# USDA-ARS-GBRU/itsxpress

Measured on AMD Instinct MI355X. Metric: reads/sec trimmed (ITS2, stand-in taxon Tracheophyta for Fungi), higher is better.
Workload: dtype u8+f32

## Files before the change

itsxpress_amd/csrc/engine.hip:

```cpp
#include <algorithm>
#include <chrono>
#include <cmath>
#include <cstdio>
#include <cstring>
#include <functional>
#include <map>
#include <memory>
#include <numeric>
#include <atomic>
#include <condition_variable>
#include <mutex>
#include <thread>
#include "detmath.h"
#include "engine.h"
#include "k_api.h"
#include "cluster_multi.h"
#include "fastq_io.h"
#include "writers.h"

namespace itsx {
void launch_region_offsets(int64_t npairs, const PairRec *pairs, const int32_t *pref, const int64_t *seg_pair_start,
                           const int64_t *seg_region_start, int64_t *pair_region0, hipStream_t st);
void launch_finalize(itsx_domain *dom, int64_t n, const int64_t *domz, double domE, const int32_t *usample, int P, hipStream_t st);
void launch_positions(const itsx_domain *dom, int64_t n, const int8_t *side, unsigned long long *bl, unsigned long long *br,
// ... 2233 lines not shown
      const int lanes_norm = waves_target <= 0 ? MR_LANES : (int)std::max<int64_t>(2, std::min<int64_t>(MR_LANES, (NU + waves_target - 1) / waves_target));
      std::vector<WaveDesc> mw;
      std::vector<int64_t> wfirst;
      for (int64_t x = 0; x < NU;) {
        const int lanes = x >= NU - n_long ? std::min(lanes_long, lanes_norm) : (int)std::min<int64_t>(lanes_norm, NU - n_long - x);
        WaveDesc d{};
        d.prof = -1; d.first = x; d.count = (int32_t)std::min<int64_t>(lanes, (int64_t)NU - x);
        d.rows = hlen[(size_t)ord[(size_t)(d.first + d.count - 1)]] + 1;
        wfirst.push_back(x);
        mw.push_back(d);
        x += d.count;
      }
      const int NMW = (int)mw.size();
      wfirst.push_back(NU);
      HIPCHK(upload(ctx->w_mrwaves, mw, st));
      const int64_t mrow_bytes = (int64_t)MRV * 16;
      const int64_t mbudget = std::max<int64_t>(1, (int64_t)(std::min(slab_gb, 16.0) * (1 << 30)) / mrow_bytes);
      const int64_t wave_cap = std::max<int64_t>(1, ((int64_t)6 << 30) / ((int64_t)MR_SCRATCH * MR_LANES));
      int w0 = 0;
      int64_t mr_wave_cap = wave_cap;
      while (w0 < NMW) {
        int w1 = w0;
        const int64_t row0 = hrow[(size_t)wfirst[(size_t)w0]];
        auto rows_to = [&](int w) { return hrow[(size_t)wfirst[(size_t)std::min(w, NMW)]] - row0; };
        while (w1 < NMW && w1 - w0 < std::min(wave_cap, mr_wave_cap) && (w1 == w0 || rows_to(w1 + 1) <= mbudget)) w1++;
        const int64_t r = rows_to(w1);
        if (((size_t)r * MRV * 4 > ctx->w_mrslab.cap && ctx->w_mrslab.alloc((size_t)r * MRV * 4) != hipSuccess) ||
            ctx->w_mrscratch.alloc((size_t)(wfirst[(size_t)w1] - wfirst[(size_t)w0]) * MR_SCRATCH) != hipSuccess) {
          (void)hipGetLastError();
          if (w1 - w0 <= 1) SET_ERR(ctx, ITSX_E_NOMEM, "no device memory left for the matrices of one wave of multidomain regions");
          mr_wave_cap = std::max<int64_t>(1, (int64_t)(w1 - w0) / 2);
          S.n_slab_shrinks++;
          continue;
        }
        MrArgs ma{};
        ma.rd = ctx->rd; ma.sorted_uniq = d_sorted; ma.seed_read = ctx->d_seed_read.p; ma.prof = ctx->d_prof.p; ma.pairs = pl.pairs;
        ma.mr = ctx->w_mr.p; ma.ulist = ulist.p; ma.u0 = wfirst[(size_t)w0]; ma.waves = ctx->w_mrwaves.p; ma.slab = (float4 *)ctx->w_mrslab.p;
        ma.rowoff = ctx->w_mrrowoff.p; ma.rowoff0 = row0;
        ma.n2off = ctx->w_n2off.p; ma.n2sc = ctx->w_n2sc.p; ma.out = ctx->w_mrout.p; ma.scratch = ctx->w_mrscratch.p;
        static const bool mrdbg = sw_get("ITSX_MR_DEBUG") != nullptr;
        if (mrdbg) { HIPCHK(ctx->w_counters.alloc(8)); HIPCHK(hipMemsetAsync(ctx->w_counters.p, 0, 64, st)); ma.dbg = (unsigned long long *)ctx->w_counters.p; }
        const int64_t one_max = sw_get("ITSX_MR_ONE_MAX") ? atoll(sw_get("ITSX_MR_ONE_MAX")) : 2048;
        const int64_t nreg = wfirst[(size_t)w1] - wfirst[(size_t)w0];
        const bool one = nreg <= one_max;
        if (one) ma.lds_bytes = (int32_t)std::min<int64_t>(40 << 10, (int64_t)mw[(size_t)w1 - 1].rows * MRV * 16);
        launch_mr_ensemble(ma, w1 - w0, w0, st, one ? wfirst[(size_t)w0] : 0, one ? nreg : 0);
        if (mrdbg) {
          unsigned long long d[5];
          HIPCHK(hipMemcpyAsync(d, ctx->w_counters.p, 40, hipMemcpyDeviceToHost, st)); HIPCHK(hipStreamSynchronize(st));
          fprintf(stderr, "[itsx] ensemble batch: %d waves, %lld matrix rows; per wave (100 MHz ticks): walk %.0f, close %.0f (samples %.0f), cluster %.0f\n", w1 - w0, (long long)r,
                  (double)d[0] / std::max<double>(1.0, (double)d[3]), (double)d[1] / std::max<double>(1.0, (double)d[3]), (double)d[4] / std::max<double>(1.0, (double)d[3]),
                  (double)d[2] / std::max<double>(1.0, (double)d[3]));
        }
        w0 = w1;
      }
      {
        HIPCHK(ctx->w_mrsel.alloc((size_t)NU + 1)); HIPCHK(ctx->w_pool_n.alloc(2));
        HIPCHK(hipMemsetAsync(ctx->w_pool_n.p + 1, 0, sizeof(unsigned long long), st));
        launch_mr_overflowed(ctx->w_mrout.p, NU, ctx->w_mrsel.p, ctx->w_pool_n.p + 1, st);
        unsigned long long nov = 0;
        HIPCHK(hipMemcpyAsync(&nov, ctx->w_pool_n.p + 1, sizeof(nov), hipMemcpyDeviceToHost, st));
        HIPCHK(hipStreamSynchronize(st));
        if (nov > 0) {
          std::vector<int32_t> sel((size_t)nov);
          HIPCHK(hipMemcpyAsync(sel.data(), ctx->w_mrsel.p, (size_t)nov * 4, hipMemcpyDeviceToHost, st));
// ... 18 lines not shown
              const int64_t bytes = al(8ll * g.capT) + 6 * al(4ll * g.capT) + al(4ll * hs) + al(4ll * g.capD) + al(16ll * g.capD) + 3 * al(4 * capSig) +
                                    al(g.capT) + al(2ll * g.capD) + al(capSig) + al(2 * MR_EPC) + 64;
              g.envoff = envoff[x1];
              if (x1 > x0 && arena + bytes > ((int64_t)8 << 30)) break;
              g.off = arena; arena += bytes;
              big.push_back(g); srow.push_back(rows); rows += Lr + 1;
              x1++;
            }
            for (size_t x = x0; x < x1; x += MR_LANES_LONG) {
              WaveDesc d{}; d.prof = -1; d.first = (int64_t)(x - x0); d.count = (int32_t)std::min<size_t>(MR_LANES_LONG, x1 - x);
              d.rows = hlen[(size_t)ord[(size_t)sel[x + d.count - 1]]] + 1;
              bw.push_back(d);
            }
            std::vector<int32_t> selb(sel.begin() + x0, sel.begin() + x1);
            HIPCHK(upload(ctx->w_mrsel, selb, st)); HIPCHK(upload(ctx->w_mrselrow, srow, st)); HIPCHK(upload(ctx->w_mrbig, big, st)); HIPCHK(upload(ctx->w_mrbigwaves, bw, st));
            if ((size_t)rows * MRV * 4 > ctx->w_mrslab.cap) HIPCHK(ctx->w_mrslab.alloc((size_t)rows * MRV * 4));
            HIPCHK(ctx->w_mrarena.alloc((size_t)arena));
            MrArgs mb{};
            mb.rd = ctx->rd; mb.sorted_uniq = d_sorted; mb.seed_read = ctx->d_seed_read.p; mb.prof = ctx->d_prof.p; mb.pairs = pl.pairs;
            mb.mr = ctx->w_mr.p; mb.ulist = ulist.p; mb.u0 = 0; mb.waves = ctx->w_mrbigwaves.p; mb.slab = (float4 *)ctx->w_mrslab.p;
            mb.rowoff = ctx->w_mrrowoff.p; mb.rowoff0 = 0; mb.n2off = ctx->w_n2off.p; mb.n2sc = ctx->w_n2sc.p; mb.out = ctx->w_mrout.p;
            mb.scratch = nullptr; mb.sel = ctx->w_mrsel.p; mb.sel_rowoff = ctx->w_mrselrow.p; mb.big = ctx->w_mrbig.p; mb.arena = ctx->w_mrarena.p; mb.envpool = ctx->w_mrenv.p;
            launch_mr_ensemble_big(mb, (int)bw.size(), st);
            x0 = x1;
          }
        }
      }
      S.ms_ensemble += tm_e.stop();
      HIPCHK(hipGetLastError());
      S.n_mr_clustered += NMR; S.n_mr_distinct += NU;
    }
  }
  DBuf<int32_t> &d_rcnt = ctx->w_rcnt, &d_rpref = ctx->w_rpref, &d_scan_tmp = ctx->w_scan2;
  HIPCHK(d_rcnt.alloc((size_t)NP + 1)); HIPCHK(d_rpref.alloc((size_t)NP + 1)); HIPCHK(d_scan_tmp.alloc((size_t)scan_tmp_elems(NP + 1)));
  HIPCHK(hipMemsetAsync(d_rcnt.p, 0, ((size_t)NP + 1) * 4, st));
// ... 2015 lines not shown
```

itsxpress_amd/csrc/k_api.h:

```cpp
#pragma once
#include "engine.h"

#include "detmath.h"
namespace itsx {

struct ReadsDev {
  const uint32_t *words;
  const int64_t  *woff;
  const int32_t  *len;
  const int64_t  *excoff;
  const uint32_t *exc;
  int64_t         n;
};

void launch_hash_reads(const ReadsDev &rd, uint64_t seed, int strand_both, uint64_t *hf, uint64_t *hr, hipStream_t st, const int32_t *sample = nullptr);
void launch_table_insert(int64_t n, const int32_t *len, int minlen, const uint64_t *hf, const uint64_t *hr,
                         unsigned long long *keys, int32_t *vals, uint64_t mask, uint32_t *slot_of, hipStream_t st);
void launch_table_resolve(const ReadsDev &rd, const uint64_t *hf, const int32_t *vals, const uint32_t *slot_of,
                          int32_t *rep_of, int8_t *strand, int32_t *is_seed, unsigned int *n_collisions, hipStream_t st,
                          const int32_t *sample = nullptr);
void launch_uniques(int64_t n, const int32_t *rep_of, const int32_t *seed_rank, int32_t *uniq_of, int32_t *seed_read,
                    int32_t *abundance, hipStream_t st);
void launch_len_hist(int32_t U, const int32_t *seed_read, const int32_t *len, int32_t *hist, int32_t lcap, hipStream_t st, int32_t nb = 0 );
void launch_len_scatter(int32_t U, const int32_t *seed_read, const int32_t *len, int32_t *cursor, int32_t lcap,
// ... 307 lines not shown

struct EnvArgs {
  ReadsDev rd;
  const int32_t *sorted_uniq, *seed_read;
  const DevProfile *prof;
  const LenTables *lt;
  const PairRec *pairs;
  const RegionRec *regions;
  RegionOut *rout;
  const WaveDesc *waves;
  float *slab;
};
void launch_envelopes(const EnvArgs &a, int nwaves, int wave0, int generic_q, hipStream_t st);

constexpr int MRV = 52;
constexpr int MRENV = 4;
#ifndef ITSX_MR_LANES
#define ITSX_MR_LANES 64
#endif
constexpr int MR_LANES = ITSX_MR_LANES;
constexpr int MR_LANES_LONG = 4;
constexpr double MR_LONG_FRAC = 0.02;
constexpr int MR_MAXD = 8;
constexpr int MR_TCAP = 512;
constexpr int MR_SCAP = 200 * MR_MAXD;
constexpr int MR_NSIG = 32;
static_assert(MR_NSIG * 50 >= 200 * MR_MAXD, "MR_NSIG must hold every cluster that can reach 25 % of 200 paths");
constexpr int MR_HASH = 1024;
constexpr int MR_EPC = 256;
constexpr int MR_SCRATCH = 19456;
struct MrRec { int32_t pair, ireg, jreg, slot; };
struct MrOut { int32_t status, nenv; int32_t ei[MRENV], ej[MRENV]; int64_t big; };
struct MrBig { int64_t off, envoff; int32_t capD, capT; uint32_t hmask; int32_t pad; };
struct MrArgs {
  ReadsDev rd;
  const int32_t *sorted_uniq, *seed_read;
  const DevProfile *prof;
  const PairRec *pairs;
  const MrRec *mr;
  const int32_t *ulist;
  int64_t u0;
  const WaveDesc *waves;
  int32_t lds_bytes = 0;
  float4 *slab;
  const int64_t *rowoff;
  int64_t rowoff0;
  const int64_t *n2off;
  float *n2sc;
  MrOut *out;
  uint8_t *scratch;
  const int32_t *sel; const int64_t *sel_rowoff; const MrBig *big; uint8_t *arena;
  int32_t *envpool;
  unsigned long long *dbg;
};
void launch_mr_count(const PairOut *pout, const RegionRec *raw, RegionPoolView pv, int64_t npairs, int32_t *cnt, hipStream_t st);
void launch_mr_fill(const PairOut *pout, const RegionRec *raw, RegionPoolView pv, int64_t npairs, const int32_t *off, MrRec *mr, hipStream_t st);
void launch_mr_ulist(int64_t nmr, const MrRec *mr, const int32_t *rep, const int32_t *is_uniq, const int32_t *urank, int32_t *ulist, int32_t *ulen,
                     int32_t *mr_u, hipStream_t st);
void launch_mr_reorder(int64_t nu, int64_t nmr, const int32_t *newpos, const int32_t *ulist_in, int32_t *ulist_out, int32_t *mr_u, hipStream_t st);
// ... 72 lines not shown
```

itsxpress_amd/csrc/k_ensemble.hip:

```cpp
#include "engine.h"
#include "k_api.h"
#include "detmath.h"
#include "k_vec.h"
#include <type_traits>

namespace itsx {

enum { tBM = 0, tMM, tIM, tDM, tMD, tMI, tII, tDD };
enum { ST_M = 1, ST_D, ST_I, ST_S, ST_N, ST_B, ST_E, ST_C, ST_T, ST_J };

DEV f4 *mrslab(const MrArgs &a, int64_t r0, int row, int v, int lane) { (void)lane; return (f4 *)a.slab + ((r0 + row) * MRV + v); }
constexpr int MR_SP = QMAX * 4 + 1, MR_CJ = QMAX * 4 + 2;
static_assert(MR_CJ < MRV, "matrix row too short");
DEV float comp4(const f4 &t, int r) { return r == 0 ? t.x : r == 1 ? t.y : r == 2 ? t.z : t.w; }
DEV f4 tof4(const V4 &v) { return (f4){v.a.x, v.a.y, v.b.x, v.b.y}; }

struct MrLane {
  bool active; int64_t mi, slot; MrRec m; int L, Lr, off, Q; const DevProfile *pp; Seq sq; float pmove, ploop; int64_t r0;
};
DEV MrLane mr_lane(const MrArgs &a, const WaveDesc &wd, int lane)
{
  MrLane e;
  e.active = lane < wd.count;
  const int64_t slot = wd.first + (e.active ? lane : 0);
// ... 102 lines not shown

DEV uint32_t rnd_mix3(uint32_t a, uint32_t b, uint32_t c)
{
  a -= b; a -= c; a ^= (c >> 13);
  b -= c; b -= a; b ^= (a << 8);
  c -= a; c -= b; c ^= (b >> 13);
  a -= b; a -= c; a ^= (c >> 12);
  b -= c; b -= a; b ^= (a << 16);
  c -= a; c -= b; c ^= (b >> 5);
  a -= b; a -= c; a ^= (c >> 3);
  b -= c; b -= a; b ^= (a << 10);
  c -= a; c -= b; c ^= (b >> 15);
  return c;
}
DEV double rng_next(uint32_t &x) { x *= 69069u; x += 1u; return (double)x / 4294967296.0; }
DEV int choose_n(uint32_t &rng, int n, float p0, float p1, float p2, float p3)
{
  float sum = 0.f; sum += p0; sum += p1; sum += p2; sum += p3;
  if (sum != 0.0f) { p0 /= sum; p1 /= sum; p2 /= sum; p3 /= sum; }
  else { p0 = p1 = (float)(1. / (double)(float)n); p2 = p3 = n == 4 ? p0 : 0.0f; }
  const double roll = rng_next(rng);
  double s = 0.0;
  s += p0; if (roll < s) return 0;
  s += p1; if (roll < s) return 1;
  s += p2; if (roll < s) return 2;
  s += p3; if (roll < s) return 3;
  int i;
  do { i = (int)(rng_next(rng) * n); } while ((i == 0 ? p0 : i == 1 ? p1 : i == 2 ? p2 : p3) == 0.f);
  return i;
}

DEV int choose2(uint32_t &rng, float p0, float p1)
{
  float sum = 0.f; sum += p0; sum += p1;
  if (sum != 0.0f) { p0 /= sum; p1 /= sum; }
  else { p0 = p1 = (float)(1. / (double)(float)2); }
  const double roll = rng_next(rng);
  double s = 0.0;
  s += p0; if (roll < s) return 0;
  s += p1; if (roll < s) return 1;
  int i;
  do { i = (int)(rng_next(rng) * 2); } while ((i == 0 ? p0 : p1) == 0.f);
  return i;
}

struct Tup { int i, j, k, m; };
DEV Tup unpack_tup(unsigned long long v) { Tup t; t.i = (int)(v & 0xffff); t.j = (int)((v >> 16) & 0xffff); t.k = (int)((v >> 32) & 0xff); t.m = (int)((v >> 40) & 0xff); return t; }
DEV unsigned long long pack_tup(int i, int j, int k, int m) { return (unsigned long long)i | ((unsigned long long)j << 16) | ((unsigned long long)k << 32) | ((unsigned long long)m << 40); }
DEV bool link_tup(const Tup &h1, const Tup &h2)
{
  int nov = min(h1.j, h2.j) - max(h1.i, h2.i) + 1;
  int n = min(h1.j - h1.i + 1, h2.j - h2.i + 1);
  if ((float)nov / (float)n < 0.8f) return false;
  nov = min(h1.m, h2.m) - max(h1.k, h2.k);
  n = min(h1.m - h1.k + 1, h2.m - h2.k + 1);
  if ((float)nov / (float)n < 0.8f) return false;
  int d1 = h1.i - h1.k, d2 = h2.i - h2.k;
  if (abs(d1 - d2) <= 4) return true;
// ... 21 lines not shown
  constexpr idx_t NONE = (idx_t)~(idx_t)0;
  constexpr int NL = ONE ? 1 : MR_LANES;
  __shared__ uint16_t cntI_s[QMAX * 4][NL];
  __shared__ uint32_t dom_ij[MR_MAXD][NL];
  __shared__ uint16_t dom_km[MR_MAXD][NL];
  __shared__ f4 dn2_one[ONE ? MR_MAXD : 1];
  WaveDesc wd;
  if constexpr (ONE) { wd.prof = -1; wd.first = wave0 + (int64_t)(gridDim.x - 1 - blockIdx.x); wd.count = 1; wd.rows = 0; }
  else wd = a.waves[wave0 + (gridDim.x - 1 - blockIdx.x)];
  const bool coop = !ONE && !BIG && wd.count <= 8;
  int P2 = 1; while (P2 < wd.count) P2 <<= 1;
  const int G = coop ? 64 / P2 : 1, hlp = coop ? (int)threadIdx.x / P2 : 0;
  const int lane = ONE ? 0 : (coop ? (int)threadIdx.x % P2 : (int)threadIdx.x);
  const MrLane e = mr_lane(a, wd, lane);
  const f4 *mat = (const f4 *)a.slab + e.r0 * MRV;
  bool in_lds = false;
  if constexpr (ONE) {
    const int64_t nvec = (int64_t)(e.Lr + 1) * MRV;
    if (nvec * 16 <= (int64_t)a.lds_bytes) {
      for (int64_t z = threadIdx.x; z < nvec; z += 64) mr_mat[z] = mat[z];
      in_lds = true;
    }
    __syncthreads();
  } else {
    if (!e.active) return;
  }
  const bool walker = ONE ? threadIdx.x == 0 : hlp == 0;
  const int tid = (int)threadIdx.x;
#define MATV(idx) ((ONE && in_lds) ? mr_mat[(idx)] : mat[(idx)])
  const int Q = e.Q, Lr = e.Lr, Lw = ONE ? e.Lr : wd.rows - 1;
  const float *tfn = e.pp->tfn;
  const float pmove = e.pmove, ploop = e.ploop;
  float *n2 = a.n2sc + a.n2off[e.mi];
  MrBig bg; bg.off = 0; bg.envoff = 0; bg.capD = MR_MAXD; bg.capT = MR_TCAP; bg.hmask = MR_HASH - 1; bg.pad = 0;
  if constexpr (BIG) bg = a.big[e.slot];
  const int capD = BIG ? bg.capD : MR_MAXD, capT = BIG ? bg.capT : MR_TCAP, capS = BIG ? bg.capT : MR_SCAP;
  const int capSig = BIG ? 4 * bg.capD : MR_NSIG, capEnv = BIG ? 4 * bg.capD : MRENV;
  const uint32_t hmask = BIG ? bg.hmask : (uint32_t)(MR_HASH - 1);
  unsigned long long *Skey; idx_t *Stcount, *Scomp, *Sstack, *Sninc, *Stid, *Shslot; sidx_t *Slast; uint8_t *Stidx, *Sdominated;
  uint16_t *Sepc; int32_t *Ssig_i, *Ssig_j, *Senv = nullptr; float *Ssig_p; f4 *Sdn2; uint32_t *Gdom_ij = nullptr; uint16_t *Gdom_km = nullptr;
  if constexpr (BIG) {
    uint8_t *blk = a.arena + bg.off;
    size_t o = 0;
    auto take = [&](size_t bytes) { uint8_t *q = blk + o; o += (bytes + 15) & ~(size_t)15; return q; };
// ... 2 lines not shown
    Sninc = (idx_t *)take(4 * (size_t)capT); Slast = (sidx_t *)take(4 * (size_t)capT); Stid = (idx_t *)take(4 * (size_t)capT);
    Shslot = (idx_t *)take(4 * ((size_t)hmask + 1));
    Gdom_ij = (uint32_t *)take(4 * (size_t)capD); Sdn2 = (f4 *)take(16 * (size_t)capD);
    Ssig_i = (int32_t *)take(4 * (size_t)capSig); Ssig_j = (int32_t *)take(4 * (size_t)capSig); Ssig_p = (float *)take(4 * (size_t)capSig);
    Senv = a.envpool + bg.envoff;
    Stidx = (uint8_t *)take((size_t)capT); Gdom_km = (uint16_t *)take(2 * (size_t)capD); Sdominated = (uint8_t *)take((size_t)capSig);
    Sepc = (uint16_t *)take(2 * MR_EPC);
  } else {
    MrScratch &S = *(MrScratch *)(a.scratch + (int64_t)(e.mi - a.u0) * MR_SCRATCH);
    Skey = S.key; Stcount = (idx_t *)S.tcount; Scomp = (idx_t *)S.comp; Sstack = (idx_t *)S.stack; Sninc = (idx_t *)S.ninc; Slast = (sidx_t *)S.last;
    Stid = (idx_t *)S.tid; Stidx = S.tidx; Shslot = (idx_t *)S.hslot; Sepc = S.epc; Ssig_i = S.sig_i; Ssig_j = S.sig_j; Ssig_p = S.sig_p;
    Sdominated = S.dominated; Sdn2 = S.dn2;
  }
#define DOM_IJ(d) (*(BIG ? &Gdom_ij[(d)] : &dom_ij[(d) < MR_MAXD ? (d) : 0][lane]))
#define DOM_KM(d) (*(BIG ? &Gdom_km[(d)] : &dom_km[(d) < MR_MAXD ? (d) : 0][lane]))
  if constexpr (ONE) {
    for (int pos = tid; pos < Lr; pos += 64) n2[pos] = 0.0f;
    for (uint32_t z = (uint32_t)tid; z <= hmask; z += 64) Shslot[z] = 0;
    __threadfence_block();
    __syncthreads();
  } else if (coop) {
    for (int pos = hlp; pos < Lr; pos += G) n2[pos] = 0.0f;
    for (uint32_t z = (uint32_t)hlp; z <= hmask; z += (uint32_t)G) Shslot[z] = 0;
    __threadfence_block();
    __syncthreads();
  } else {
    for (int pos = 0; pos < Lr; pos++) n2[pos] = 0.0f;
    for (uint32_t z = 0; z <= hmask; z++) Shslot[z] = 0;
  }
  uint32_t rng = rnd_mix3(42u, 87654321u, 12345678u);
  if (rng == 0) rng = 42;
  int ntup = 0, nsamp = 0, status = walker ? 0 : 9;
  const unsigned short dgm[16] = {1, 2, 4, 8, 0, 5, 10, 3, 12, 6, 9, 11, 14, 7, 13, 15};
  int ex0p = -1, ex0c = 0, ex1p = -1, ex1c = 0;
  if (e.sq.nexc >= 1 && e.sq.nexc <= 2) { const uint32_t v = e.sq.exc[0]; ex0p = (int)(v >> 4); ex0c = (int)(v & 15u); }
  if (e.sq.nexc == 2) { const uint32_t v = e.sq.exc[1]; ex1p = (int)(v >> 4); ex1c = (int)(v & 15u); }

  unsigned long long tk_walk = 0, tk_close = 0, tk_dedupe = 0;
  for (int t = 0; t < 200; t++) {
    if (__ballot(status == 0) == 0ull) break;
    const unsigned long long tk0 = wall_clock64();
    int i = Lr, k = 0, s0 = status == 0 ? ST_C : ST_S, nd = 0;
    int cj_row = -1; f4 cj_cur = (f4){0.f, 0.f, 0.f, 0.f};
    int dfrom = 0, dto = 0, dk = 0, dm = 0;
    unsigned long long maskM = 0ull;
    while (__ballot(s0 != ST_S) != 0ull) {
      while (__ballot(s0 == ST_C || s0 == ST_J) != 0ull) {
        if (!(s0 == ST_C || s0 == ST_J)) continue;
        if (i < 1) { status = 5; s0 = ST_S; continue; }
        if (cj_row != i) { cj_cur = MATV((int64_t)i * MRV + MR_CJ); cj_row = i; }
        const f4 c0 = MATV((int64_t)(i - 1) * MRV + MR_CJ);
        const float w0 = (s0 == ST_C ? c0.z : c0.y) * ploop, w1 = cj_cur.x * 0.5f * cj_cur.w;
        if (choose2(rng, w0, w1) == 0) { i--; cj_cur = c0; cj_row = i; } else s0 = ST_E;
      }
      if (__ballot(s0 == ST_E) != 0ull) {
        if (s0 == ST_E) {
          double sum = 0.0;
          const double roll = rng_next(rng);
          const double norm = 1.0 / (double)cj_cur.x;
          const float xEv = (float)norm;
          int s1 = -1;
          while (s1 < 0) {
            for (int q0 = 0; q0 < Q && s1 < 0; q0 += 3) {
              f2 md[3][4];
#pragma unroll
              for (int z = 0; z < 3; z++) {
                const int qq = q0 + z < Q ? q0 + z : Q - 1;
#pragma unroll
                for (int rr = 0; rr < 4; rr++) { const f4 q4 = MATV((int64_t)i * MRV + (rr * Q + qq + 1)); md[z][rr] = (f2){q4.x, q4.y}; }
              }
#pragma unroll
              for (int z = 0; z < 3; z++) {
                if (q0 + z >= Q || s1 >= 0) continue;
                const int qq = q0 + z;
#pragma unroll
                for (int rr = 0; rr < 4; rr++) { if (s1 < 0) { sum += (double)(md[z][rr].x * xEv); if (roll < sum) { k = rr * Q + qq + 1; s1 = ST_M; } } }
// ... 4 lines not shown
            if (s1 < 0 && sum < 0.99) { status = 1; s1 = ST_S; }
          }
          if (status == 0 && nd >= capD) { status = 2; s1 = ST_S; }
          if (status == 0) {
            nd++;
            dfrom = dto = dk = dm = 0;
            maskM = 0ull;
            for (int z = 0; z < Q * 4; z++) cntI_s[z][lane] = 0;
            if (s1 == ST_M) { dto = i; dm = k; dfrom = i; dk = k; maskM |= 1ull << k; }
          }
          s0 = s1;
        }
      }
      while (__ballot(s0 == ST_M || s0 == ST_D || s0 == ST_I) != 0ull) {
        if (!(s0 == ST_M || s0 == ST_D || s0 == ST_I)) continue;
        const int rowA = (s0 == ST_D) ? i : i - 1;
        const int kA = (s0 == ST_I) ? k : k - 1;
        const f4 nv = MATV((int64_t)rowA * MRV + kA);
        const f4 tv = *(const f4 *)(tfn + (s0 == ST_D ? kA : k) * 8 + (s0 == ST_M ? 0 : 4));
        float w0, w1, w2 = 0.0f, w3 = 0.0f;
        if (s0 == ST_M) { w0 = nv.w * tv.x; w1 = nv.x * tv.y; w2 = nv.z * tv.z; w3 = nv.y * tv.w; }
        else if (s0 == ST_D) { w0 = nv.x * tv.x; w1 = nv.y * tv.w; }
        else { w0 = nv.x * tv.y; w1 = nv.z * tv.z; }
        const int c = choose_n(rng, s0 == ST_M ? 4 : 2, w0, w1, w2, w3);
        int s1;
        if (s0 == ST_M) { s1 = c == 0 ? ST_B : c == 1 ? ST_M : c == 2 ? ST_I : ST_D; k--; i--; }
        else if (s0 == ST_D) { s1 = c == 0 ? ST_M : ST_D; k--; }
        else { s1 = c == 0 ? ST_M : ST_I; i--; }
        if (s1 == ST_M) {
          if (dto == 0) { dto = i; dm = k; }
          dfrom = i; dk = k;
          maskM |= 1ull << k;
        } else if (s1 == ST_I) {
          cntI_s[k - 1][lane] += 1;
        }
        s0 = s1;
      }
      if (__ballot(s0 == ST_B) != 0ull) {
        if (s0 == ST_B) {
          const f4 sp1 = MATV((int64_t)i * MRV + MR_SP);
          s0 = choose2(rng, sp1.y * pmove, sp1.z * pmove) == 0 ? ST_S : ST_J;
          int Ld = __popcll(maskM);
          for (int z = 0; z < Q * 4; z++) Ld += (int)cntI_s[z][lane];
          const float norm = (float)(1.0 / (double)(float)Ld);
          const float xfactor = (0.0f * norm + 0.0f * norm) + 0.0f * norm;
          V4 sv[4];
#pragma unroll
          for (int x = 0; x < 4; x++) sv[x] = vzero();
          for (int qq = 0; qq < Q; qq++) {
            V4 mv, iv;
            mv.a = (f2){(float)((maskM >> (0 * Q + qq + 1)) & 1ull), (float)((maskM >> (1 * Q + qq + 1)) & 1ull)};
            mv.b = (f2){(float)((maskM >> (2 * Q + qq + 1)) & 1ull), (float)((maskM >> (3 * Q + qq + 1)) & 1ull)};
            iv.a = (f2){(float)cntI_s[0 * Q + qq][lane], (float)cntI_s[1 * Q + qq][lane]}; iv.b = (f2){(float)cntI_s[2 * Q + qq][lane], (float)cntI_s[3 * Q + qq][lane]};
            mv = vmul(mv, vset(norm)); iv = vmul(iv, vset(norm));
#pragma unroll
            for (int x = 0; x < 4; x++) {
// ... 267 lines not shown
      }
    for (int d = 0; d < nsig; d++) {
      if (Sdominated[d]) continue;
      if (out.nenv >= capEnv) { status = 7; break; }
      if (out.nenv < MRENV) { out.ei[out.nenv] = Ssig_i[d]; out.ej[out.nenv] = Ssig_j[d]; }
      if constexpr (BIG) { Senv[2 * out.nenv] = Ssig_i[d]; Senv[2 * out.nenv + 1] = Ssig_j[d]; }
      out.nenv++;
    }
  }
  if (status != 0) {
    out.nenv = 0;
    for (int pos = 0; pos < Lr; pos++) n2[pos] = 0.0f;
  }
  out.status = status;
  a.out[e.mi] = out;
  if (a.dbg && lane == 0) { atomicAdd(&a.dbg[0], tk_walk); atomicAdd(&a.dbg[1], tk_close); atomicAdd(&a.dbg[2], wall_clock64() - tk2); atomicAdd(&a.dbg[3], 1ull); atomicAdd(&a.dbg[4], tk_dedupe); }
}
#undef DOM_IJ
#undef DOM_KM

__global__ void __launch_bounds__(256) k_mr_count(const PairOut *__restrict__ pout, const RegionRec *__restrict__ raw, RegionPoolView pv, int64_t npairs,
                                                  int32_t *__restrict__ cnt)
{
  const int64_t pi = (int64_t)blockIdx.x * blockDim.x + threadIdx.x;
  if (pi > npairs) return;
  int c = 0;
  if (pi < npairs && pout[pi].pass_fwd)
    for (int k = 0; k < pout[pi].ndom; k++) c += raw_region(raw, pv, pi, k).multi != 0;
  cnt[pi] = c;
}
__global__ void __launch_bounds__(256) k_mr_fill(const PairOut *__restrict__ pout, const RegionRec *__restrict__ raw, RegionPoolView pv, int64_t npairs,
                                                 const int32_t *__restrict__ off, MrRec *__restrict__ mr)
{
  const int64_t pi = (int64_t)blockIdx.x * blockDim.x + threadIdx.x;
// ... 105 lines not shown
                     int32_t *mr_u, hipStream_t st)
{
  if (nmr <= 0) return;
  hipLaunchKernelGGL(k_mr_ulist, dim3((unsigned)((nmr + 255) / 256)), dim3(256), 0, st, nmr, mr, rep, is_uniq, urank, ulist, ulen, mr_u);
}
void launch_mr_reorder(int64_t nu, int64_t nmr, const int32_t *newpos, const int32_t *ulist_in, int32_t *ulist_out, int32_t *mr_u, hipStream_t st)
{
  const int64_t n = nu > nmr ? nu : nmr;
  if (n <= 0) return;
  hipLaunchKernelGGL(k_mr_reorder, dim3((unsigned)((n + 255) / 256)), dim3(256), 0, st, nu, nmr, newpos, ulist_in, ulist_out, mr_u);
}
void launch_mr_ensemble(const MrArgs &a, int nwaves, int wave0, hipStream_t st, int64_t one_first, int64_t one_count)
{
  if (nwaves <= 0) return;
  hipLaunchKernelGGL(k_mr_fwd, dim3(nwaves), dim3(64), 0, st, a, wave0);
  if (one_count > 0) hipLaunchKernelGGL((k_mr_trace<false, true>), dim3((unsigned)one_count), dim3(64), (size_t)a.lds_bytes, st, a, (int)one_first);
  else hipLaunchKernelGGL(k_mr_trace<false>, dim3(nwaves), dim3(64), 0, st, a, wave0);
}
void launch_mr_ensemble_big(const MrArgs &a, int nwaves, hipStream_t st)
{
  if (nwaves <= 0) return;
  hipLaunchKernelGGL(k_mr_fwd, dim3(nwaves), dim3(64), 0, st, a, 0);
  hipLaunchKernelGGL(k_mr_trace<true>, dim3(nwaves), dim3(64), 0, st, a, 0);
}
}
```

itsxpress_amd/csrc/switches.cpp:

```cpp
#include "switches.h"
#include <cstdlib>
#include <cstring>

namespace itsx {

static const Switch g_sw[] = {
  {"ITSX_NO_ENSEMBLE", SW_HOOK, "multidomain regions keep their region as one envelope instead of hmmsearch's stochastic-traceback clustering (changes envelopes)"},
  {"ITSX_LAZY_ZUB_SCALE", SW_HOOK, "multiplies the lazy stage's upper bound on domZ: more undecided rows for the completion tests"},
  {"ITSX_LAZY_FORCE_PENDING", SW_HOOK, "treats rows as undecided so that the completion path runs"},
  {"ITSX_LAZY_NO_RERUN", SW_HOOK, "skips the full re-search safety net (leaves undecided rows undecided)"},
  {"ITSX_LAZY_NO_COMPLETE", SW_HOOK, "skips itsx_lazy_complete inside itsx_search_finalize (leaves undecided rows undecided)"},
  {"ITSX_COMPACT_ZMAX", SW_HOOK, "largest domZ the compact / lazy modes call a row 'certain' for (default 1e9); a value below the data's domZ can drop a winner"},
  {"ITSX_COMPACT_DOME_MIN", SW_HOOK, "smallest --domE the compact / lazy modes call a row 'certain' for (default 1e-2)"},
  {"ITSX_PASSA_DBG", SW_HOOK, "pass A diagnostic bits (no rows / no restore / no join): timings only, scores are garbage"},
  {"ITSX_ROWS", SW_MODE, "rows mode when the caller did not call itsx_set_rows_mode: full | compact | lazy (coordinates identical in all three)"},
  {"ITSX_COMPACT_ROWS", SW_MODE, "=1: rows mode compact (older spelling of ITSX_ROWS=compact)"},
  {"ITSX_QMASK", SW_MODE, "=none: vsearch's --qmask none for cluster_size / orient seeds (default dust, as vsearch)"},
  {"ITSX_KEEP_TRACE", SW_MODE, "keeps per-pair filter traces for itsx_get_pairtraces (forces the compact path of a lazy search)"},
  {"ITSX_GZIP_LEVEL", SW_MODE, "deflate level of the trimmed-FASTQ writers (default 6; output bytes differ, records do not)"},
  {"ITSX_TEST_HOOKS", SW_DIAG, "=1: honour the HOOK switches above"},
  {"ITSX_SHARE_CHECK", SW_DIAG, "runs the unshared kernels beside the shared ones and counts differences (itsx_stats.share_mismatch, join_maxdiff)"},
  {"ITSX_LAZY_CHECK_BOUND", SW_DIAG, "compares pass A's scores with HMMER's own Forward arithmetic (itsx_stats.lazy_bound_maxdiff)"},
  {"ITSX_LAZY_HIST", SW_DIAG, "prints the histogram of round-2 candidates per group"},
  {"ITSX_PASSA_DUMP", SW_DIAG, "prints every pass-A launch's waves and wave-rows (scripts/passa_launches.py)"},
// ... 17 lines not shown
  {"ITSX_MSV_OVERLAP", SW_TUNING, "=0: the next chunk's MSV filter does not run beside the domain stage"},
  {"ITSX_MSV_PAD", SW_TUNING, "dynamic LDS of the overlapped MSV launch (an occupancy cap)"},
  {"ITSX_MSV_WHOLE", SW_TUNING, "=0: MSV stages 16 words at a time even when the whole read fits LDS"},
  {"ITSX_BIAS_OVERLAP", SW_TUNING, "=0: the bias filter does not run on the second stream"},
  {"ITSX_ST2_PRIO", SW_TUNING, "priority of the second stream"},
  {"ITSX_LOAD_PRIORITY", SW_TUNING, "=0: loads do not use the high-priority stream"},
  {"ITSX_SLAB_GB", SW_TUNING, "DP slab budget, GB"},
  {"ITSX_SLAB_ADAPT", SW_TUNING, "=0: the slab budget does not adapt to the job"},
  {"ITSX_DEFER_FREE_GB", SW_TUNING, "device memory kept on the deferred-free list, GB"},
  {"ITSX_MR_LONG_FRAC", SW_TUNING, "ensemble stage: share of regions taken as 'long'"},
  {"ITSX_MR_LONG_LANES", SW_TUNING, "ensemble stage: lanes per long region"},
  {"ITSX_MSV_BWD_WHOLE", SW_TUNING, "=1: the MSV filter's Backward chains copy their whole read to LDS first (A/B arm: same cells)"},
  {"ITSX_LAZY_TOPUP_ALL", SW_TUNING, "=0: a profile whose undecided rows need most of its pairs is left to the full count (itsx_lazy_complete) instead of taking all its unevaluated pairs in the top-up round (same rows)"},
  {"ITSX_MR_WAVES", SW_TUNING, "ensemble stage: waves a batch is spread over (lanes per wave = regions / this, 2 .. 64); 0 = waves of 64 lanes"},
  {"ITSX_MR_ONE_MAX", SW_TUNING, "ensemble stage: a batch of at most this many regions (default 2048) is walked one region per wave with the matrix in LDS; 0 = never"},
  {"ITSX_CL_NOSCORE", SW_TUNING, "clustering: skips the score-only pre-pass (A/B arm; the walk then aligns every candidate: same outcomes)"},
  {"ITSX_CL_NOPRECHECK", SW_TUNING, "clustering: skips the certificate pre-check (A/B arm: same outcomes)"},
  {"ITSX_CL_CAPACITY", SW_TUNING, "clustering: candidate-list capacity"},
  {"ITSX_CL_CCAP", SW_TUNING, "clustering: centroid capacity step"},
  {"ITSX_CL_HEAVY", SW_TUNING, "clustering: heavy-word split on / off"},
  {"ITSX_CL_HEAVY_MIN", SW_TUNING, "clustering: centroids a word needs to count as conserved"},
  {"ITSX_CL_ROWS", SW_TUNING, "clustering: alignment rows per lane"},
  {"ITSX_CL_WINDOW", SW_TUNING, "clustering: queries per speculative window"},
  {"ITSX_PACK_CHUNK", SW_TUNING, "reads per packing launch"},
  {"ITSX_PACK_ECAP", SW_TUNING, "initial capacity of the exception list"},
  {"ITSX_HUGEPAGES", SW_TUNING, "=0: host buffers without MADV_HUGEPAGE"},
  {"ITSX_IO_LIBDEFLATE", SW_TUNING, "=0: zlib instead of libdeflate when both are present"},
  {"ITSX_IO_THREADS", SW_TUNING, "host threads of the FASTQ readers / writers"},
  {"ITSX_IO_BLOCK_KB", SW_TUNING, "deflate unit of the block-parallel writer"},
  {"ITSX_PARALLEL_INFLATE", SW_TUNING, "=0: single-stream inflate"},
// ... 39 lines not shown
```

Baseline: 4.588 million.

## Precompute per-region normalized choice table for ensemble stochastic traceback walkers

Before the stochastic traceback walk, each region's helper lanes now fill a table of pre-normalised transition probabilities (M, D/I, emission, C/J, B choices) held in extra slab space. The walker then reads these probabilities directly instead of multiplying matrix entries by transitions and normalising at every step. The serial walker does less work per step, and the table fill is spread across lanes. In exchange the slab grows per row, the one-region-per-wave path gives up its LDS matrix copy when the table is on, and every cell is filled even if the walk never visits it. It is on by default for waves of at most 8 lanes and for the overflow path.

```diff
diff --git a/itsxpress_amd/csrc/engine.hip b/itsxpress_amd/csrc/engine.hip
--- a/itsxpress_amd/csrc/engine.hip
+++ b/itsxpress_amd/csrc/engine.hip
@@ -2271,7 +2271,11 @@
       const int NMW = (int)mw.size();
       wfirst.push_back(NU);
       HIPCHK(upload(ctx->w_mrwaves, mw, st));
-      const int64_t mrow_bytes = (int64_t)MRV * 16;
+      const char *mrt_sw = sw_get("ITSX_MR_TABLE");
+      const bool mr_table = mrt_sw ? atoi(mrt_sw) != 0 : lanes_norm <= 8;
+      const bool mr_table_big = mrt_sw ? atoi(mrt_sw) != 0 : true;
+      const int64_t mr_rowv = MRV + (mr_table ? MRT : 0), mr_rowv_big = MRV + (mr_table_big ? MRT : 0);
+      const int64_t mrow_bytes = mr_rowv * 16;
       const int64_t mbudget = std::max<int64_t>(1, (int64_t)(std::min(slab_gb, 16.0) * (1 << 30)) / mrow_bytes);
       const int64_t wave_cap = std::max<int64_t>(1, ((int64_t)6 << 30) / ((int64_t)MR_SCRATCH * MR_LANES));
       int w0 = 0;
@@ -2282,7 +2286,7 @@
         auto rows_to = [&](int w) { return hrow[(size_t)wfirst[(size_t)std::min(w, NMW)]] - row0; };
         while (w1 < NMW && w1 - w0 < std::min(wave_cap, mr_wave_cap) && (w1 == w0 || rows_to(w1 + 1) <= mbudget)) w1++;
         const int64_t r = rows_to(w1);
-        if (((size_t)r * MRV * 4 > ctx->w_mrslab.cap && ctx->w_mrslab.alloc((size_t)r * MRV * 4) != hipSuccess) ||
+        if (((size_t)r * mr_rowv * 4 > ctx->w_mrslab.cap && ctx->w_mrslab.alloc((size_t)r * mr_rowv * 4) != hipSuccess) ||
             ctx->w_mrscratch.alloc((size_t)(wfirst[(size_t)w1] - wfirst[(size_t)w0]) * MR_SCRATCH) != hipSuccess) {
           (void)hipGetLastError();
           if (w1 - w0 <= 1) SET_ERR(ctx, ITSX_E_NOMEM, "no device memory left for the matrices of one wave of multidomain regions");
@@ -2293,6 +2297,7 @@
         MrArgs ma{};
         ma.rd = ctx->rd; ma.sorted_uniq = d_sorted; ma.seed_read = ctx->d_seed_read.p; ma.prof = ctx->d_prof.p; ma.pairs = pl.pairs;
         ma.mr = ctx->w_mr.p; ma.ulist = ulist.p; ma.u0 = wfirst[(size_t)w0]; ma.waves = ctx->w_mrwaves.p; ma.slab = (float4 *)ctx->w_mrslab.p;
+        ma.tab = mr_table ? (float4 *)ctx->w_mrslab.p + (size_t)r * MRV : nullptr;
         ma.rowoff = ctx->w_mrrowoff.p; ma.rowoff0 = row0;
         ma.n2off = ctx->w_n2off.p; ma.n2sc = ctx->w_n2sc.p; ma.out = ctx->w_mrout.p; ma.scratch = ctx->w_mrscratch.p;
         static const bool mrdbg = sw_get("ITSX_MR_DEBUG") != nullptr;
@@ -2303,9 +2308,10 @@
         if (one) ma.lds_bytes = (int32_t)std::min<int64_t>(40 << 10, (int64_t)mw[(size_t)w1 - 1].rows * MRV * 16);
         launch_mr_ensemble(ma, w1 - w0, w0, st, one ? wfirst[(size_t)w0] : 0, one ? nreg : 0);
         if (mrdbg) {
-          unsigned long long d[5];
-          HIPCHK(hipMemcpyAsync(d, ctx->w_counters.p, 40, hipMemcpyDeviceToHost, st)); HIPCHK(hipStreamSynchronize(st));
-          fprintf(stderr, "[itsx] ensemble batch: %d waves, %lld matrix rows; per wave (100 MHz ticks): walk %.0f, close %.0f (samples %.0f), cluster %.0f\n", w1 - w0, (long long)r,
+          unsigned long long d[6];
+          HIPCHK(hipMemcpyAsync(d, ctx->w_counters.p, 48, hipMemcpyDeviceToHost, st)); HIPCHK(hipStreamSynchronize(st));
+          fprintf(stderr, "[itsx] ensemble batch: %d waves, %lld regions, %lld matrix rows; per wave (100 MHz ticks): table %.0f, walk %.0f, close %.0f (samples %.0f), cluster %.0f\n", w1 - w0, (long long)nreg, (long long)r,
+                  (double)d[5] / std::max<double>(1.0, (double)d[3]),
                   (double)d[0] / std::max<double>(1.0, (double)d[3]), (double)d[1] / std::max<double>(1.0, (double)d[3]), (double)d[4] / std::max<double>(1.0, (double)d[3]),
                   (double)d[2] / std::max<double>(1.0, (double)d[3]));
         }
@@ -2354,11 +2360,12 @@
             }
             std::vector<int32_t> selb(sel.begin() + x0, sel.begin() + x1);
             HIPCHK(upload(ctx->w_mrsel, selb, st)); HIPCHK(upload(ctx->w_mrselrow, srow, st)); HIPCHK(upload(ctx->w_mrbig, big, st)); HIPCHK(upload(ctx->w_mrbigwaves, bw, st));
-            if ((size_t)rows * MRV * 4 > ctx->w_mrslab.cap) HIPCHK(ctx->w_mrslab.alloc((size_t)rows * MRV * 4));
+            if ((size_t)rows * mr_rowv_big * 4 > ctx->w_mrslab.cap) HIPCHK(ctx->w_mrslab.alloc((size_t)rows * mr_rowv_big * 4));
             HIPCHK(ctx->w_mrarena.alloc((size_t)arena));
             MrArgs mb{};
             mb.rd = ctx->rd; mb.sorted_uniq = d_sorted; mb.seed_read = ctx->d_seed_read.p; mb.prof = ctx->d_prof.p; mb.pairs = pl.pairs;
             mb.mr = ctx->w_mr.p; mb.ulist = ulist.p; mb.u0 = 0; mb.waves = ctx->w_mrbigwaves.p; mb.slab = (float4 *)ctx->w_mrslab.p;
+            mb.tab = mr_table_big ? (float4 *)ctx->w_mrslab.p + (size_t)rows * MRV : nullptr;
             mb.rowoff = ctx->w_mrrowoff.p; mb.rowoff0 = 0; mb.n2off = ctx->w_n2off.p; mb.n2sc = ctx->w_n2sc.p; mb.out = ctx->w_mrout.p;
             mb.scratch = nullptr; mb.sel = ctx->w_mrsel.p; mb.sel_rowoff = ctx->w_mrselrow.p; mb.big = ctx->w_mrbig.p; mb.arena = ctx->w_mrarena.p; mb.envpool = ctx->w_mrenv.p;
             launch_mr_ensemble_big(mb, (int)bw.size(), st);
diff --git a/itsxpress_amd/csrc/k_api.h b/itsxpress_amd/csrc/k_api.h
--- a/itsxpress_amd/csrc/k_api.h
+++ b/itsxpress_amd/csrc/k_api.h
@@ -345,6 +345,12 @@
 void launch_envelopes(const EnvArgs &a, int nwaves, int wave0, int generic_q, hipStream_t st);
 
 constexpr int MRV = 52;
+constexpr int MRT_M = 0;
+constexpr int MRT_DI = QMAX * 4 + 1;
+constexpr int MRT_E = 2 * (QMAX * 4 + 1);
+constexpr int MRT_CJ = MRT_E + 2 * QMAX;
+constexpr int MRT_B = MRT_CJ + 1;
+constexpr int MRT = MRT_B + 1;
 constexpr int MRENV = 4;
 #ifndef ITSX_MR_LANES
 #define ITSX_MR_LANES 64
@@ -374,6 +380,7 @@
   const WaveDesc *waves;
   int32_t lds_bytes = 0;
   float4 *slab;
+  float4 *tab;
   const int64_t *rowoff;
   int64_t rowoff0;
   const int64_t *n2off;
diff --git a/itsxpress_amd/csrc/k_ensemble.hip b/itsxpress_amd/csrc/k_ensemble.hip
--- a/itsxpress_amd/csrc/k_ensemble.hip
+++ b/itsxpress_amd/csrc/k_ensemble.hip
@@ -140,11 +140,15 @@
   return c;
 }
 DEV double rng_next(uint32_t &x) { x *= 69069u; x += 1u; return (double)x / 4294967296.0; }
-DEV int choose_n(uint32_t &rng, int n, float p0, float p1, float p2, float p3)
+DEV f4 fnorm_n(int n, float p0, float p1, float p2, float p3)
 {
   float sum = 0.f; sum += p0; sum += p1; sum += p2; sum += p3;
   if (sum != 0.0f) { p0 /= sum; p1 /= sum; p2 /= sum; p3 /= sum; }
   else { p0 = p1 = (float)(1. / (double)(float)n); p2 = p3 = n == 4 ? p0 : 0.0f; }
+  return (f4){p0, p1, p2, p3};
+}
+DEV int fchoose_n(uint32_t &rng, int n, float p0, float p1, float p2, float p3)
+{
   const double roll = rng_next(rng);
   double s = 0.0;
   s += p0; if (roll < s) return 0;
@@ -155,12 +159,21 @@
   do { i = (int)(rng_next(rng) * n); } while ((i == 0 ? p0 : i == 1 ? p1 : i == 2 ? p2 : p3) == 0.f);
   return i;
 }
-
-DEV int choose2(uint32_t &rng, float p0, float p1)
+DEV int choose_n(uint32_t &rng, int n, float p0, float p1, float p2, float p3)
+{
+  const f4 p = fnorm_n(n, p0, p1, p2, p3);
+  return fchoose_n(rng, n, p.x, p.y, p.z, p.w);
+}
+
+DEV f2 fnorm2(float p0, float p1)
 {
   float sum = 0.f; sum += p0; sum += p1;
   if (sum != 0.0f) { p0 /= sum; p1 /= sum; }
   else { p0 = p1 = (float)(1. / (double)(float)2); }
+  return (f2){p0, p1};
+}
+DEV int fchoose2(uint32_t &rng, float p0, float p1)
+{
   const double roll = rng_next(rng);
   double s = 0.0;
   s += p0; if (roll < s) return 0;
@@ -168,6 +181,56 @@
   int i;
   do { i = (int)(rng_next(rng) * 2); } while ((i == 0 ? p0 : p1) == 0.f);
   return i;
+}
+DEV int choose2(uint32_t &rng, float p0, float p1)
+{
+  const f2 p = fnorm2(p0, p1);
+  return fchoose2(rng, p.x, p.y);
+}
+
+DEV void mr_fill_table(f4 *__restrict__ tab, const f4 *__restrict__ mat, const float *__restrict__ tfn, int Q, int Lr, float pmove, float ploop,
+                       int first, int step)
+{
+  const int K1 = Q * 4 + 1;
+  const int ncell = (Lr + 1) * K1;
+#pragma unroll 2
+  for (int c = first; c < ncell; c += step) {
+    const int i = c / K1, k = c - i * K1;
+    if (k == 0) continue;
+    const f4 cur = mat[(int64_t)i * MRV + (k - 1)];
+    const f4 tD = *(const f4 *)(tfn + (k - 1) * 8 + 4);
+    const f4 pd = fnorm_n(2, cur.x * tD.x, cur.y * tD.w, 0.0f, 0.0f);
+    f4 pm = fnorm_n(4, 0.0f, 0.0f, 0.0f, 0.0f), pi = fnorm_n(2, 0.0f, 0.0f, 0.0f, 0.0f);
+    if (i >= 1) {
+      const f4 up = mat[(int64_t)(i - 1) * MRV + (k - 1)], upk = mat[(int64_t)(i - 1) * MRV + k];
+      const f4 tM = *(const f4 *)(tfn + k * 8), tI = *(const f4 *)(tfn + k * 8 + 4);
+      pm = fnorm_n(4, up.w * tM.x, up.x * tM.y, up.z * tM.z, up.y * tM.w);
+      pi = fnorm_n(2, upk.x * tI.y, upk.z * tI.z, 0.0f, 0.0f);
+    }
+    tab[(int64_t)i * MRT + MRT_M + k] = pm;
+    tab[(int64_t)i * MRT + MRT_DI + k] = (f4){pd.x, pd.y, pi.x, pi.y};
+  }
+  for (int c = first; c < Lr * Q; c += step) {
+    const int i = c / Q + 1, q = c - (i - 1) * Q;
+    const float xEv = (float)(1.0 / (double)mat[(int64_t)i * MRV + MR_CJ].x);
+    const f4 n0 = mat[(int64_t)i * MRV + (0 * Q + q + 1)], n1 = mat[(int64_t)i * MRV + (1 * Q + q + 1)];
+    const f4 n2 = mat[(int64_t)i * MRV + (2 * Q + q + 1)], n3 = mat[(int64_t)i * MRV + (3 * Q + q + 1)];
+    tab[(int64_t)i * MRT + MRT_E + 2 * q] = (f4){n0.x * xEv, n1.x * xEv, n2.x * xEv, n3.x * xEv};
+    tab[(int64_t)i * MRT + MRT_E + 2 * q + 1] = (f4){n0.y * xEv, n1.y * xEv, n2.y * xEv, n3.y * xEv};
+  }
+  for (int i = first; i <= Lr; i += step) {
+    const f4 sp = mat[(int64_t)i * MRV + MR_SP];
+    const f2 pb = fnorm2(sp.y * pmove, sp.z * pmove);
+    f2 pc = fnorm2(0.0f, 0.0f), pj = pc;
+    if (i >= 1) {
+      const f4 c0 = mat[(int64_t)(i - 1) * MRV + MR_CJ], ci = mat[(int64_t)i * MRV + MR_CJ];
+      const float w1 = ci.x * 0.5f * ci.w;
+      pc = fnorm2(c0.z * ploop, w1);
+      pj = fnorm2(c0.y * ploop, w1);
+    }
+    tab[(int64_t)i * MRT + MRT_CJ] = (f4){pc.x, pc.y, pj.x, pj.y};
+    tab[(int64_t)i * MRT + MRT_B] = (f4){pb.x, pb.y, 0.0f, 0.0f};
+  }
 }
 
 struct Tup { int i, j, k, m; };
@@ -219,10 +282,12 @@
   const int lane = ONE ? 0 : (coop ? (int)threadIdx.x % P2 : (int)threadIdx.x);
   const MrLane e = mr_lane(a, wd, lane);
   const f4 *mat = (const f4 *)a.slab + e.r0 * MRV;
+  const bool use_tab = a.tab != nullptr;
+  f4 *tabr = use_tab ? (f4 *)a.tab + e.r0 * MRT : nullptr;
   bool in_lds = false;
   if constexpr (ONE) {
     const int64_t nvec = (int64_t)(e.Lr + 1) * MRV;
-    if (nvec * 16 <= (int64_t)a.lds_bytes) {
+    if (!use_tab && nvec * 16 <= (int64_t)a.lds_bytes) {
       for (int64_t z = threadIdx.x; z < nvec; z += 64) mr_mat[z] = mat[z];
       in_lds = true;
     }
@@ -233,6 +298,7 @@
   const bool walker = ONE ? threadIdx.x == 0 : hlp == 0;
   const int tid = (int)threadIdx.x;
 #define MATV(idx) ((ONE && in_lds) ? mr_mat[(idx)] : mat[(idx)])
+#define TABV(row, v) (tabr[(int64_t)(row) * MRT + (v)])
   const int Q = e.Q, Lr = e.Lr, Lw = ONE ? e.Lr : wd.rows - 1;
   const float *tfn = e.pp->tfn;
   const float pmove = e.pmove, ploop = e.ploop;
@@ -265,19 +331,15 @@
   }
 #define DOM_IJ(d) (*(BIG ? &Gdom_ij[(d)] : &dom_ij[(d) < MR_MAXD ? (d) : 0][lane]))
 #define DOM_KM(d) (*(BIG ? &Gdom_km[(d)] : &dom_km[(d) < MR_MAXD ? (d) : 0][lane]))
-  if constexpr (ONE) {
-    for (int pos = tid; pos < Lr; pos += 64) n2[pos] = 0.0f;
-    for (uint32_t z = (uint32_t)tid; z <= hmask; z += 64) Shslot[z] = 0;
+  const int sfirst = ONE ? tid : hlp, sstep = ONE ? 64 : G;
+  for (int pos = sfirst; pos < Lr; pos += sstep) n2[pos] = 0.0f;
+  for (uint32_t z = (uint32_t)sfirst; z <= hmask; z += (uint32_t)sstep) Shslot[z] = 0;
+  const unsigned long long tkf0 = wall_clock64();
+  if (use_tab) mr_fill_table(tabr, mat, tfn, Q, Lr, pmove, ploop, sfirst, sstep);
+  const unsigned long long tk_fill = wall_clock64() - tkf0;
+  if (ONE || coop) {
     __threadfence_block();
     __syncthreads();
-  } else if (coop) {
-    for (int pos = hlp; pos < Lr; pos += G) n2[pos] = 0.0f;
-    for (uint32_t z = (uint32_t)hlp; z <= hmask; z += (uint32_t)G) Shslot[z] = 0;
-    __threadfence_block();
-    __syncthreads();
-  } else {
-    for (int pos = 0; pos < Lr; pos++) n2[pos] = 0.0f;
-    for (uint32_t z = 0; z <= hmask; z++) Shslot[z] = 0;
   }
   uint32_t rng = rnd_mix3(42u, 87654321u, 12345678u);
   if (rng == 0) rng = 42;
@@ -299,6 +361,11 @@
       while (__ballot(s0 == ST_C || s0 == ST_J) != 0ull) {
         if (!(s0 == ST_C || s0 == ST_J)) continue;
         if (i < 1) { status = 5; s0 = ST_S; continue; }
+        if (use_tab) {
+          const f4 cj = TABV(i, MRT_CJ);
+          if (fchoose2(rng, s0 == ST_C ? cj.x : cj.z, s0 == ST_C ? cj.y : cj.w) == 0) i--; else s0 = ST_E;
+          continue;
+        }
         if (cj_row != i) { cj_cur = MATV((int64_t)i * MRV + MR_CJ); cj_row = i; }
         const f4 c0 = MATV((int64_t)(i - 1) * MRV + MR_CJ);
         const float w0 = (s0 == ST_C ? c0.z : c0.y) * ploop, w1 = cj_cur.x * 0.5f * cj_cur.w;
@@ -308,9 +375,29 @@
         if (s0 == ST_E) {
           double sum = 0.0;
           const double roll = rng_next(rng);
-          const double norm = 1.0 / (double)cj_cur.x;
+          const double norm = use_tab ? 0.0 : 1.0 / (double)cj_cur.x;
           const float xEv = (float)norm;
           int s1 = -1;
+          while (use_tab && s1 < 0) {
+            for (int q0 = 0; q0 < Q && s1 < 0; q0 += 3) {
+              f4 em[3], ed[3];
+#pragma unroll
+              for (int z = 0; z < 3; z++) {
+                const int qq = q0 + z < Q ? q0 + z : Q - 1;
+                em[z] = TABV(i, MRT_E + 2 * qq); ed[z] = TABV(i, MRT_E + 2 * qq + 1);
+              }
+#pragma unroll
+              for (int z = 0; z < 3; z++) {
+                if (q0 + z >= Q || s1 >= 0) continue;
+                const int qq = q0 + z;
+#pragma unroll
+                for (int rr = 0; rr < 4; rr++) { if (s1 < 0) { sum += (double)comp4(em[z], rr); if (roll < sum) { k = rr * Q + qq + 1; s1 = ST_M; } } }
+#pragma unroll
+                for (int rr = 0; rr < 4; rr++) { if (s1 < 0) { sum += (double)comp4(ed[z], rr); if (roll < sum) { k = rr * Q + qq + 1; s1 = ST_D; } } }
+              }
+            }
+            if (s1 < 0 && sum < 0.99) { status = 1; s1 = ST_S; }
+          }
           while (s1 < 0) {
             for (int q0 = 0; q0 < Q && s1 < 0; q0 += 3) {
               f2 md[3][4];
@@ -345,15 +432,22 @@
       }
       while (__ballot(s0 == ST_M || s0 == ST_D || s0 == ST_I) != 0ull) {
         if (!(s0 == ST_M || s0 == ST_D || s0 == ST_I)) continue;
-        const int rowA = (s0 == ST_D) ? i : i - 1;
-        const int kA = (s0 == ST_I) ? k : k - 1;
-        const f4 nv = MATV((int64_t)rowA * MRV + kA);
-        const f4 tv = *(const f4 *)(tfn + (s0 == ST_D ? kA : k) * 8 + (s0 == ST_M ? 0 : 4));
-        float w0, w1, w2 = 0.0f, w3 = 0.0f;
-        if (s0 == ST_M) { w0 = nv.w * tv.x; w1 = nv.x * tv.y; w2 = nv.z * tv.z; w3 = nv.y * tv.w; }
-        else if (s0 == ST_D) { w0 = nv.x * tv.x; w1 = nv.y * tv.w; }
-        else { w0 = nv.x * tv.y; w1 = nv.z * tv.z; }
-        const int c = choose_n(rng, s0 == ST_M ? 4 : 2, w0, w1, w2, w3);
+        int c;
+        if (use_tab) {
+          if (i < 1 && s0 != ST_D) { status = 5; s0 = ST_S; continue; }
+          const f4 pv = TABV(i, (s0 == ST_M ? MRT_M : MRT_DI) + k);
+          c = fchoose_n(rng, s0 == ST_M ? 4 : 2, s0 == ST_I ? pv.z : pv.x, s0 == ST_I ? pv.w : pv.y, s0 == ST_M ? pv.z : 0.0f, s0 == ST_M ? pv.w : 0.0f);
+        } else {
+          const int rowA = (s0 == ST_D) ? i : i - 1;
+          const int kA = (s0 == ST_I) ? k : k - 1;
+          const f4 nv = MATV((int64_t)rowA * MRV + kA);
+          const f4 tv = *(const f4 *)(tfn + (s0 == ST_D ? kA : k) * 8 + (s0 == ST_M ? 0 : 4));
+          float w0, w1, w2 = 0.0f, w3 = 0.0f;
+          if (s0 == ST_M) { w0 = nv.w * tv.x; w1 = nv.x * tv.y; w2 = nv.z * tv.z; w3 = nv.y * tv.w; }
+          else if (s0 == ST_D) { w0 = nv.x * tv.x; w1 = nv.y * tv.w; }
+          else { w0 = nv.x * tv.y; w1 = nv.z * tv.z; }
+          c = choose_n(rng, s0 == ST_M ? 4 : 2, w0, w1, w2, w3);
+        }
         int s1;
         if (s0 == ST_M) { s1 = c == 0 ? ST_B : c == 1 ? ST_M : c == 2 ? ST_I : ST_D; k--; i--; }
         else if (s0 == ST_D) { s1 = c == 0 ? ST_M : ST_D; k--; }
@@ -369,8 +463,8 @@
       }
       if (__ballot(s0 == ST_B) != 0ull) {
         if (s0 == ST_B) {
-          const f4 sp1 = MATV((int64_t)i * MRV + MR_SP);
-          s0 = choose2(rng, sp1.y * pmove, sp1.z * pmove) == 0 ? ST_S : ST_J;
+          if (use_tab) { const f4 pb = TABV(i, MRT_B); s0 = fchoose2(rng, pb.x, pb.y) == 0 ? ST_S : ST_J; }
+          else { const f4 sp1 = MATV((int64_t)i * MRV + MR_SP); s0 = choose2(rng, sp1.y * pmove, sp1.z * pmove) == 0 ? ST_S : ST_J; }
           int Ld = __popcll(maskM);
           for (int z = 0; z < Q * 4; z++) Ld += (int)cntI_s[z][lane];
           const float norm = (float)(1.0 / (double)(float)Ld);
@@ -668,10 +762,12 @@
   }
   out.status = status;
   a.out[e.mi] = out;
-  if (a.dbg && lane == 0) { atomicAdd(&a.dbg[0], tk_walk); atomicAdd(&a.dbg[1], tk_close); atomicAdd(&a.dbg[2], wall_clock64() - tk2); atomicAdd(&a.dbg[3], 1ull); atomicAdd(&a.dbg[4], tk_dedupe); }
+  if (a.dbg && lane == 0) { atomicAdd(&a.dbg[0], tk_walk); atomicAdd(&a.dbg[1], tk_close); atomicAdd(&a.dbg[2], wall_clock64() - tk2); atomicAdd(&a.dbg[3], 1ull); atomicAdd(&a.dbg[4], tk_dedupe); atomicAdd(&a.dbg[5], tk_fill); }
 }
 #undef DOM_IJ
 #undef DOM_KM
+#undef MATV
+#undef TABV
 
 __global__ void __launch_bounds__(256) k_mr_count(const PairOut *__restrict__ pout, const RegionRec *__restrict__ raw, RegionPoolView pv, int64_t npairs,
                                                   int32_t *__restrict__ cnt)
@@ -807,7 +903,7 @@
 {
   if (nwaves <= 0) return;
   hipLaunchKernelGGL(k_mr_fwd, dim3(nwaves), dim3(64), 0, st, a, wave0);
-  if (one_count > 0) hipLaunchKernelGGL((k_mr_trace<false, true>), dim3((unsigned)one_count), dim3(64), (size_t)a.lds_bytes, st, a, (int)one_first);
+  if (one_count > 0) hipLaunchKernelGGL((k_mr_trace<false, true>), dim3((unsigned)one_count), dim3(64), a.tab ? 0 : (size_t)a.lds_bytes, st, a, (int)one_first);
   else hipLaunchKernelGGL(k_mr_trace<false>, dim3(nwaves), dim3(64), 0, st, a, wave0);
 }
 void launch_mr_ensemble_big(const MrArgs &a, int nwaves, hipStream_t st)
diff --git a/itsxpress_amd/csrc/switches.cpp b/itsxpress_amd/csrc/switches.cpp
--- a/itsxpress_amd/csrc/switches.cpp
+++ b/itsxpress_amd/csrc/switches.cpp
@@ -55,6 +55,7 @@
   {"ITSX_LAZY_TOPUP_ALL", SW_TUNING, "=0: a profile whose undecided rows need most of its pairs is left to the full count (itsx_lazy_complete) instead of taking all its unevaluated pairs in the top-up round (same rows)"},
   {"ITSX_MR_WAVES", SW_TUNING, "ensemble stage: waves a batch is spread over (lanes per wave = regions / this, 2 .. 64); 0 = waves of 64 lanes"},
   {"ITSX_MR_ONE_MAX", SW_TUNING, "ensemble stage: a batch of at most this many regions (default 2048) is walked one region per wave with the matrix in LDS; 0 = never"},
+  {"ITSX_MR_TABLE", SW_TUNING, "ensemble stage: =0: the walker normalises a step's candidates itself instead of reading the region's choice table (A/B arm: same draws, same bits); =1: the table also for waves of 64 regions (default: waves of at most 8 and the overflow path)"},
   {"ITSX_CL_NOSCORE", SW_TUNING, "clustering: skips the score-only pre-pass (A/B arm; the walk then aligns every candidate: same outcomes)"},
   {"ITSX_CL_NOPRECHECK", SW_TUNING, "clustering: skips the certificate pre-check (A/B arm: same outcomes)"},
   {"ITSX_CL_CAPACITY", SW_TUNING, "clustering: candidate-list capacity"},
```

After: 4.610 million (median of 6 runs). About the same (+0.5%).
